# ZhonghuaYi/EI-Nexus_official

Measured on AMD Instinct MI355X. Metric: event-image pairs/s (extract+match, 346x260, 1024 kpts), higher is better.
Workload: dtype f32; 1 GPU; B32 346x260 5-bin event voxel + gray image, VGG(event)+SuperPoint(image) extractors, MNN matcher, k=1024; global_batch=32, event_bins=5, parallelism=dp1 (pairs sharded, metric all-reduce only), log_assignment=False, dense_outputs=False, same_scene_pairs=False, weights=seeded synthetic, descriptor-head bias calibrated (per-channel mean removed)

## Files before the change

### ei-nexus_official_amd/_lib.py

```python
import ctypes
import os

_HERE = os.path.dirname(os.path.abspath(__file__))
LIB_PATH = os.environ.get("EINX_LIB") or os.path.join(_HERE, "libeinx_hip.so")

c_void_p, c_int, c_float, c_size_t, c_char_p = ctypes.c_void_p, ctypes.c_int, ctypes.c_float, ctypes.c_size_t, ctypes.c_char_p


class ConvDesc(ctypes.Structure):
    _fields_ = [("w_native", c_void_p), ("bias", c_void_p), ("scale", c_void_p), ("shift", c_void_p),
                ("cin", ctypes.c_int32), ("cout", ctypes.c_int32), ("ks", ctypes.c_int32), ("relu", ctypes.c_int32),
                ("pool", ctypes.c_int32)]


class DetectParams(ctypes.Structure):
    _fields_ = [("B", ctypes.c_int32), ("Hp", ctypes.c_int32), ("Wp", ctypes.c_int32), ("H", ctypes.c_int32),
                ("W", ctypes.c_int32), ("h0", ctypes.c_int32), ("w0", ctypes.c_int32), ("radius", ctypes.c_int32),
                ("top_k", ctypes.c_int32), ("det_thr", c_float), ("ordering_xy", ctypes.c_int32), ("cap", ctypes.c_int32),
                ("nms_iters", ctypes.c_int32)]


class ExtractorDesc(ctypes.Structure):
    _fields_ = [("struct_size", c_size_t), ("cell", ctypes.c_int32), ("n_backbone", ctypes.c_int32), ("n_det", ctypes.c_int32), ("n_desc", ctypes.c_int32),
                ("backbone", ctypes.POINTER(ConvDesc)), ("det_head", ctypes.POINTER(ConvDesc)), ("desc_head", ctypes.POINTER(ConvDesc)),
# ... 52 lines not shown
                ("match_w", c_void_p), ("match_b", c_void_p), ("n_layers", ctypes.c_int32), ("heads", ctypes.c_int32),
                ("d", ctypes.c_int32), ("input_dim", ctypes.c_int32), ("filter_threshold", c_float),
                ("layers", ctypes.POINTER(LgLayer))]


class LgHead(ctypes.Structure):
    _fields_ = [(n, c_void_p) for n in ("proj_w", "proj_b", "match_w", "match_b", "token_w", "token_b")]


SIGNATURES = {
    "einx_version": (c_char_p, []),
    "einx_abi_version": (c_int, []),
    "einx_build_flags": (c_char_p, []),
    "einx_params_hash": (c_int, [c_void_p, c_int, c_void_p, c_void_p, c_void_p, c_void_p]),
    "einx_last_error": (c_char_p, []),
    "einx_math_eval": (c_int, [c_int, c_void_p, ctypes.c_longlong, c_void_p, c_void_p]),
    "einx_fork_stream_of": (c_void_p, [c_void_p]),
    "einx_fork_stream_prepare_beside": (c_int, [c_void_p, ctypes.POINTER(c_void_p), c_int]),
    "einx_stream_overlap_us": (c_int, [c_void_p, c_void_p, c_int, ctypes.POINTER(ctypes.c_float)]),
    "einx_device_count": (c_int, []),
    "einx_profile_enable": (c_int, [c_int]),
    "einx_profile_report": (c_int, [c_char_p, c_size_t]),
    "einx_extractor_create": (c_void_p, [ctypes.POINTER(ExtractorDesc)]),
    "einx_extractor_destroy": (None, [c_void_p]),
    "einx_fork_stream_prepare": (c_int, [c_void_p]),
    "einx_fork_stream_release": (c_int, [c_void_p]),
    "einx_fork_stream_count": (c_int, []),
    "einx_side_stream": (c_void_p, [c_void_p, c_int, ctypes.POINTER(c_void_p), c_int]),
    "einx_extract_shapes": (c_int, [c_void_p, c_int, c_int, ctypes.POINTER(ExtractShapes)]),
    "einx_extract_ws_bytes": (c_size_t, [c_void_p, c_int, c_int, c_int, c_int, c_int]),
    "einx_extract": (c_int, [c_void_p, c_void_p, c_void_p, c_int, c_int, c_int, c_int, c_void_p, c_size_t, ctypes.POINTER(ExtractOut), c_void_p]),
    "einx_extract_watch": (c_int, [c_void_p, c_void_p, c_void_p, c_int, c_int, c_int, c_int, c_void_p, c_size_t, ctypes.POINTER(ExtractOut),
                           ctypes.POINTER(WeightWatch), c_void_p]),
    "einx_conv_last_kernel": (c_char_p, []),
    "einx_conv_weight_elems": (c_size_t, [c_int, c_int, c_int]),
    "einx_conv_repack": (c_int, [c_void_p, c_int, c_int, c_int, c_void_p, c_void_p]),
    "einx_bn_fold": (c_int, [c_void_p, c_void_p, c_void_p, c_void_p, c_float, c_int, c_void_p, c_void_p, c_void_p]),
    "einx_conv_block": (c_int, [c_void_p, c_int, c_int, c_int, c_int, c_int, c_int, c_int, ctypes.POINTER(ConvDesc), c_void_p, c_void_p]),
    "einx_conv_first_two_fused_ok": (c_int, [ctypes.POINTER(ConvDesc), ctypes.POINTER(ConvDesc), c_int, c_int, c_int]),
    "einx_conv_first_two_fused": (c_int, [c_void_p, c_int, c_int, c_int, c_int, c_int, c_int, c_int, ctypes.POINTER(ConvDesc), ctypes.POINTER(ConvDesc),
                                  c_void_p, c_void_p]),
    "einx_div_inplace": (c_int, [c_void_p, c_size_t, c_float, c_void_p]),
    "einx_image_prepare": (c_int, [c_void_p, c_int, c_int, c_int, c_int, ctypes.c_longlong, ctypes.c_longlong, ctypes.c_longlong, ctypes.c_longlong,
                           c_float, c_void_p, c_void_p]),
    "einx_score_map": (c_int, [c_void_p, c_int, c_int, c_int, c_int, c_void_p, c_int, c_int, c_int, c_int, c_int, c_int, c_void_p,
                               c_void_p, c_void_p]),
    "einx_remove_border": (c_int, [c_void_p, c_int, c_int, c_int, c_int, c_void_p]),
    "einx_detect_ws_bytes": (c_size_t, [ctypes.POINTER(DetectParams)]),
    "einx_detect": (c_int, [c_void_p, ctypes.POINTER(DetectParams), c_void_p, c_void_p, c_void_p, c_void_p, c_void_p, c_void_p,
                            c_void_p, c_void_p]),
    "einx_desc_sample": (c_int, [c_void_p, c_int, c_int, c_int, c_int, c_int, c_int, c_int, c_int, c_void_p, c_void_p, c_int, c_float,
                                 c_void_p, c_void_p]),
    "einx_normalize_map": (c_int, [c_void_p, c_int, c_int, c_int, c_float, c_void_p, c_void_p, c_void_p]),
    "einx_upsample_ws_bytes": (c_size_t, [c_int, c_int, c_int]),
    "einx_upsample_normalize": (c_int, [c_void_p, c_int, c_int, c_int, c_int, c_int, c_int, c_int, c_int, c_int, c_int, c_float,
                                        c_void_p, c_void_p, c_size_t, c_void_p]),
    "einx_mnn_ws_bytes": (c_size_t, [c_int, c_int, c_int]),
    "einx_mnn": (c_int, [c_void_p, c_void_p, c_int, c_void_p, c_void_p, c_int, c_int, c_int, c_void_p, c_void_p, c_void_p, c_void_p,
                         c_void_p, c_void_p, c_void_p]),
    "einx_mnn_gather": (c_int, [c_void_p, c_void_p, c_int, c_void_p, c_void_p, c_int, c_int, c_int, c_void_p, c_void_p, c_void_p, c_void_p,
                                c_void_p, c_void_p, c_void_p, c_void_p, c_int, c_void_p, c_void_p, c_void_p, c_void_p]),
    "einx_mnn_thresh": (c_int, [c_void_p, c_void_p, c_int, c_void_p, c_void_p, c_int, c_int, c_int, c_int, c_float, c_int, c_float, c_void_p,
                                c_void_p, c_void_p, c_void_p, c_void_p, c_void_p, c_void_p]),
    "einx_gather_matches": (c_int, [c_void_p, c_void_p, c_void_p, c_void_p, c_int, c_int, c_int, c_int, c_void_p, c_void_p, c_void_p,
                                    c_void_p]),
    "einx_events_ws_bytes": (c_size_t, [c_int, c_int, c_int]),
    "einx_voxel_ws_bytes": (c_size_t, [c_int, c_int, c_int, c_int, ctypes.c_int64]),
    "einx_voxel_grid": (c_int, [c_void_p, c_void_p, c_void_p, c_void_p, c_void_p, c_int, c_int, c_int, c_int, c_int, c_void_p, c_void_p,
                                c_size_t, c_void_p]),
    "einx_events_mask": (c_int, [c_void_p, c_void_p, c_void_p, c_int, c_int, c_int, c_void_p, c_void_p, c_void_p]),
    "einx_time_surface_ws_bytes": (c_size_t, [c_int, c_int, c_int, c_int, ctypes.c_int64]),
    "einx_event_stack_ws_bytes": (c_size_t, [c_int, c_int, c_int, c_int, ctypes.c_int64]),
    "einx_distance_map_ws_bytes": (c_size_t, [c_int, c_int, c_int, c_int, ctypes.c_int64]),
    "einx_time_surface": (c_int, [c_void_p, c_void_p, c_void_p, c_void_p, c_void_p, c_int, c_int, c_int, c_int, c_void_p, c_void_p, c_size_t,
                                  c_void_p]),
    "einx_event_stack": (c_int, [c_void_p, c_void_p, c_void_p, c_void_p, c_void_p, c_int, c_int, c_int, c_int, c_void_p, c_void_p, c_size_t,
                                 c_void_p]),
    "einx_distance_map": (c_int, [c_void_p, c_void_p, c_void_p, c_void_p, c_void_p, c_int, c_int, c_int, c_int, c_void_p, c_void_p, c_size_t,
                                  c_void_p]),
    "einx_events_pack": (c_int, [ctypes.POINTER(EventArrays), c_int, c_void_p, c_void_p, c_void_p, c_void_p, c_void_p, c_int]),
    "einx_metrics_ws_bytes": (c_size_t, [ctypes.POINTER(MetricParams)]),
    "einx_pair_metrics": (c_int, [ctypes.POINTER(MetricParams)] + [c_void_p] * 13),
    "einx_relative_pose_ws_bytes": (c_size_t, [ctypes.POINTER(PoseParams)]),
    "einx_relative_pose": (c_int, [ctypes.POINTER(PoseParams)] + [c_void_p] * 13),
    "einx_essential_5pt": (c_int, [c_void_p, c_void_p, c_int, c_void_p, c_void_p, c_void_p]),
    "einx_homography_ws_bytes": (c_size_t, [ctypes.POINTER(HomographyParams)]),
    "einx_homography": (c_int, [ctypes.POINTER(HomographyParams)] + [c_void_p] * 11),
    "einx_homography_dlt": (c_int, [c_void_p, c_void_p, c_int, c_int, c_void_p, c_void_p, c_void_p]),
    "einx_gt_matches_ws_bytes": (c_size_t, [ctypes.POINTER(GtMatchesParams)]),
    "einx_gt_project": (c_int, [ctypes.POINTER(GtMatchesParams)] + [c_void_p] * 23),
    "einx_gt_warp": (c_int, [ctypes.POINTER(GtMatchesParams)] + [c_void_p] * 8),
    "einx_gt_label": (c_int, [ctypes.POINTER(GtMatchesParams)] + [c_void_p] * 17),
    "einx_gt_matches": (c_int, [ctypes.POINTER(GtMatchesParams)] + [c_void_p] * 30),
    "einx_match_pr": (c_int, [c_void_p, c_void_p, c_void_p, c_void_p, c_int, c_int, c_void_p, c_void_p]),
    "einx_desc_loss_ws_bytes": (c_size_t, [c_int] * 11),
    "einx_desc_loss": (c_int, [c_void_p, c_float, c_void_p, c_float] + [c_int] * 11 + [c_void_p, c_int, c_int, c_void_p, c_void_p, c_size_t, c_void_p]),
    "einx_map_loss_ws_bytes": (c_size_t, [c_int, c_int]),
    "einx_map_loss": (c_int, [c_void_p, c_void_p, c_int, c_int, c_int, c_void_p, c_int, c_int, c_int, c_void_p, c_void_p, c_size_t, c_void_p]),
    "einx_logits_loss": (c_int, [c_void_p, c_void_p] + [c_int] * 9 + [c_void_p, c_int, c_void_p, c_void_p, c_size_t, c_void_p]),
    "einx_linear": (c_int, [c_void_p, c_int, c_int, c_void_p, c_void_p, c_int, c_void_p, c_int, c_void_p]),
    "einx_lg_ws_bytes": (c_size_t, [c_int, c_int, c_int, c_int, c_int]),
    "einx_lg_ws_bytes_heads": (c_size_t, [c_int, c_int, c_int, c_int, c_int, c_int]),
    "einx_lightglue": (c_int, [ctypes.POINTER(LgWeights), c_void_p, c_void_p, c_void_p, c_int, c_void_p, c_void_p, c_void_p, c_int,
                               c_int, c_float, c_float, c_float, c_float, c_void_p, c_void_p, c_void_p, c_void_p, c_void_p, c_void_p,
                               c_void_p, c_void_p, c_int, c_void_p]),
    "einx_lightglue_early_stop_ws_bytes": (c_size_t, [c_int] * 7),
# ... 48 lines not shown
```

### ei-nexus_official_amd/_native.py

```python
import ctypes
import threading
import os
import math

import numpy as np
import torch

from . import _lib
from ._lib import ConvDesc, DetectParams, check

F32 = torch.float32


def lib():
    return _lib.load()


I32, I64, U8 = torch.int32, torch.int64, torch.uint8


def _dev_check(*tensors, dt=F32):
    for t in tensors:
        if t is None:
            continue
# ... 192 lines not shown

class Detection:
    __slots__ = ("positions", "indices", "counts", "thr", "not_converged", "nms", "cap", "padded", "pads", "stale")


def detect(score, *, top_k, radius, det_thr, pads=(0, 0, 0, 0), ordering="yx", cap=None, nms_iters=8, want_nms=True):
    _dev_check(score)
    B = score.shape[0]
    Hp, Wp = score.shape[-2:]
    w0, w1, h0, h1 = pads
    H, W = Hp - h0 - h1, Wp - w0 - w1
    N = Hp * Wp
    if cap is None:
        cap = topk_capacity(N, top_k, det_thr)
    cap = max(int(cap), 1)
    p = DetectParams(B, Hp, Wp, H, W, h0, w0, int(radius), int(top_k or 0), float(det_thr), int(ordering == "xy"), cap, int(nms_iters))
    L = lib()
    dev = score.device
    ws = _workspace(L.einx_detect_ws_bytes(ctypes.byref(p)), dev)
    d = Detection()
    d.positions = torch.empty((B, cap, 3), dtype=F32, device=dev)
    d.indices = torch.empty((B, cap), dtype=torch.int32, device=dev)
    d.counts = torch.empty((B,), dtype=torch.int32, device=dev)
    d.thr = torch.empty((B,), dtype=F32, device=dev)
    d.not_converged = torch.empty((B,), dtype=torch.int32, device=dev)
    d.nms = torch.empty((B, H, W), dtype=F32, device=dev) if want_nms else None
    d.cap, d.padded, d.pads = cap, (Hp, Wp), pads
    check(L.einx_detect(_ptr(score), ctypes.byref(p), _ptr(ws), _ptr(d.nms), _ptr(d.positions), _ptr(d.indices), _ptr(d.counts),
                        _ptr(d.thr), _ptr(d.not_converged), _stream(score)), "einx_detect")
    return d


def desc_sample(raw, indices, counts, padded_size, bilinear, scale, raw_cl=None):
    _dev_check(raw, raw_cl)
    _dev_check(indices, counts, dt=I32)
    B, D, hc, wc = raw.shape
    cap = indices.shape[1]
    out = torch.empty((B, cap, D), dtype=F32, device=raw.device)
    use_cl = raw_cl is not None and bilinear
    src = raw_cl if use_cl else raw
    check(lib().einx_desc_sample(_ptr(src), B, D, hc, wc, int(padded_size[0]), int(padded_size[1]), int(bilinear), int(use_cl),
                                 _ptr(indices), _ptr(counts), cap, float(scale), _ptr(out), _stream(raw)), "einx_desc_sample")
    return out


def normalize_map(raw, scale, want_cl=False):
    _dev_check(raw)
    B, D = raw.shape[:2]
    P = int(raw.numel() // (B * D))
    out = torch.empty_like(raw)
    cl = torch.empty((B, P, D), dtype=F32, device=raw.device) if (want_cl and D <= 512) else None
    check(lib().einx_normalize_map(_ptr(raw), B, D, P, float(scale), _ptr(out), _ptr(cl), _stream(raw)), "einx_normalize_map")
    return (out, cl) if want_cl else out


def upsample_normalize(raw, padded_size, pads, scale):
    _dev_check(raw)
    B, D, hc, wc = raw.shape
    Hp, Wp = int(padded_size[0]), int(padded_size[1])
    w0, w1, h0, h1 = pads
    H, W = Hp - h0 - h1, Wp - w0 - w1
    out = torch.empty((B, D, H, W), dtype=F32, device=raw.device)
    nws = int(lib().einx_upsample_ws_bytes(B, H, W))
    ws = torch.empty((nws + 3) // 4, dtype=F32, device=raw.device)
    check(lib().einx_upsample_normalize(_ptr(raw), B, D, hc, wc, Hp, Wp, h0, w0, H, W, float(scale), _ptr(out), _ptr(ws), nws, _stream(raw)),
          "einx_upsample_normalize")
    return out


class MatchResult:
    __slots__ = ("matches0", "matches1", "scores0", "scores1", "la", "mk0", "mk1", "nmatch", "ref0", "ref1", "mk0_flat", "mk1_flat", "stale", "stop")

    def __init__(self):
        self.mk0_flat = self.mk1_flat = None
        self.stale = None
        self.stop = None


def mnn(desc0, n, desc1, m, want_la=True, ratio_thresh=None, distance_thresh=None, gather=None):
    _dev_check(desc0, desc1)
    _dev_check(n, m, dt=I32)
    B, cap0, D = desc0.shape
    cap1 = desc1.shape[1]
    L = lib()
    dev = desc0.device
    ws = _workspace(L.einx_mnn_ws_bytes(B, cap0, cap1), dev)
    r = MatchResult()
    r.matches0 = torch.empty((B, cap0), dtype=torch.int64, device=dev)
    r.matches1 = torch.empty((B, cap1), dtype=torch.int64, device=dev)
    r.scores0 = torch.empty((B, cap0), dtype=F32, device=dev)
    r.scores1 = torch.empty((B, cap1), dtype=F32, device=dev)
    r.la = torch.empty((B, cap0 + 1, cap1 + 1), dtype=F32, device=dev) if want_la else None
    r.ref0 = r.ref1 = None
    if ratio_thresh or distance_thresh:
        r2 = float(np.float32(float(ratio_thresh) ** 2)) if ratio_thresh else 0.0
        t2 = float(np.float32(float(distance_thresh) ** 2)) if distance_thresh else 0.0
        check(L.einx_mnn_thresh(_ptr(desc0), _ptr(n), cap0, _ptr(desc1), _ptr(m), cap1, B, D, int(bool(ratio_thresh)), r2,
                                int(bool(distance_thresh)), t2, _ptr(ws), _ptr(r.matches0), _ptr(r.matches1), _ptr(r.scores0), _ptr(r.scores1),
                                _ptr(r.la), _stream(desc0)), "einx_mnn_thresh")
        return r if gather is None else gather_matches(r, gather[0], gather[1], n, gather[2])
    if gather is not None:
        k0, k1, cols = gather
        _dev_check(k0, k1)
        r.mk0 = torch.empty((B, cap0, cols), dtype=F32, device=dev)
        r.mk1 = torch.empty((B, cap0, cols), dtype=F32, device=dev)
        r.nmatch = torch.empty((B,), dtype=torch.int32, device=dev)
# ... 293 lines not shown
```

### ei-nexus_official_amd/csrc/extract.hip

```cpp
#include <stdlib.h>
#include <string.h>

#include <algorithm>
#include <mutex>
#include <new>
#include <vector>

#include "einx_common.h"

struct einx_extractor {
  einx_extractor_desc d;
  std::vector<einx_conv_desc> backbone, det, desc;
  bool has_merged = false;
  einx_conv_desc merged;
};

namespace {

struct Plan {
  int Hp, Wp, h0, w0;
  int hc, wc;
  size_t buf_elems[2];
  size_t head_elems;
};
// ... 182 lines not shown
                                   size_t ws_bytes, const einx_extract_out* o, const einx_weight_watch* ww, void* stream) {
  EINX_CHECK_ARG(e && in && ws && o, "null pointer");
  EINX_CHECK_ARG(!ww || ww->struct_size == sizeof(einx_weight_watch), "einx_weight_watch::struct_size does not match this library (ABI mismatch)");
  EINX_CHECK_ARG(!ww || ww->n == 0 || (ww->n > 0 && ww->table && ww->ref && ww->scratch && ww->stale), "weight watch with null pointers");
  EINX_CHECK_ARG(o->feats && o->logits && o->raw && o->prob && o->score && o->positions && o->indices && o->counts && o->thr &&
                     o->not_converged && o->sparse_desc,
                 "null output pointer");
  EINX_CHECK_ARG(B > 0 && H > 0 && W > 0 && o->cap > 0, "bad shape");
  Plan pl;
  EINX_CHECK_ARG(make_plan(e, H, W, &pl), "image size does not fit the network's pooling / cell size");
  EINX_CHECK_ARG(e->d.cell == 1 || (o->coarse && o->raw_cl), "cell-8 networks need the coarse / raw_cl outputs");
  EINX_CHECK_ARG(ws_bytes >= einx_extract_ws_bytes(e, B, H, W, o->cap, nms_iters), "workspace smaller than einx_extract_ws_bytes for these arguments");
  einx_detect_params dp;
  detect_params(e, pl, B, H, W, o->cap, nms_budget(nms_iters), &dp);
  WsCarver c{(char*)ws};
  const ExtractWs wk = carve(c, e, pl, &dp, B);
  bool fork = fork_heads(e, pl, B) && !einx_profile_active();
  {
    hipStreamCaptureStatus cs = hipStreamCaptureStatusNone;
    if (fork && hipStreamIsCapturing((hipStream_t)stream, &cs) == hipSuccess && cs != hipStreamCaptureStatusNone) fork = false;
  }
  float* const head2 = fork ? wk.head2 : wk.head;
  int rc;
  if (e->d.input_div != 0.0f && e->d.input_div != 1.0f) {
    rc = einx_div_inplace(in, (size_t)B * e->backbone.front().cin * H * W, e->d.input_div, stream);
    if (rc) return rc;
  }
  const float* cur = in;
  int h = pl.Hp, w = pl.Wp;
  const int nb = (int)e->backbone.size();
  int first = 0;
  if (nb >= 2 && 1 == einx_conv_first_two_fused_ok(&e->backbone[0], &e->backbone[1], B, pl.Hp, pl.Wp)) {
    float* out = (2 < nb) ? wk.buf[1] : o->feats;
    if ((rc = einx_conv_first_two_fused(in, B, H, W, pl.h0, pl.w0, pl.Hp, pl.Wp, &e->backbone[0], &e->backbone[1], out, stream))) return rc;
    if (e->backbone[1].pool) {
      h /= 2;
      w /= 2;
    }
    cur = out;
    first = 2;
  }
  for (int i = first; i < nb; ++i) {
    const einx_conv_desc& c = e->backbone[i];
    float* out = (i + 1 < nb) ? wk.buf[i & 1] : o->feats;
    if (i == 0) rc = einx_conv_block(cur, B, H, W, pl.h0, pl.w0, pl.Hp, pl.Wp, &c, out, stream);
    else rc = einx_conv_block(cur, B, h, w, 0, 0, h, w, &c, out, stream);
    if (rc) return rc;
    if (c.pool) {
      h /= 2;
      w /= 2;
    }
    cur = out;
  }
  auto run_head = [&](const std::vector<einx_conv_desc>& L, float* scratch, float* final_out, void* st) -> int {
    const float* x = o->feats;
    for (size_t i = 0; i < L.size(); ++i) {
      float* out = (i + 1 < L.size()) ? scratch : final_out;
      const int r = einx_conv_block(x, B, h, w, 0, 0, h, w, &L[i], out, st);
      if (r) return r;
      x = out;
    }
    return 0;
  };
  const int D = e->desc.back().cout;
  const bool merged = e->has_merged && B == 1;
  if (merged && (rc = einx_conv_block(o->feats, B, h, w, 0, 0, h, w, &e->merged, wk.head, stream))) return rc;
  const float* desc_in = wk.head + (size_t)e->det.front().cout * h * w;
  auto det_branch = [&](void* st) -> int {
    if (merged) return einx_conv_block(wk.head, B, h, w, 0, 0, h, w, &e->det[1], o->logits, st);
    return run_head(e->det, wk.head, o->logits, st);
  };
  auto desc_branch = [&](void* st) -> int {
    int r = merged ? einx_conv_block(desc_in, B, h, w, 0, 0, h, w, &e->desc[1], o->raw, st) : run_head(e->desc, head2, o->raw, st);
    if (r) return r;
    if (e->d.cell == 8) r = einx_normalize_map(o->raw, B, D, h * w, e->d.desc_scale, o->coarse, o->raw_cl, st);
    return r;
  };
  std::unique_lock<std::mutex> side_lock;
  const EinxSide* sd = fork ? einx_side_acquire((hipStream_t)stream, &side_lock) : nullptr;
  if (sd) {
    if (hipEventRecord(sd->fork, (hipStream_t)stream) != hipSuccess || hipStreamWaitEvent(sd->stream, sd->fork, 0) != hipSuccess) {
      einx_set_error("einx_extract: fork failed");
      return EINX_ERR_LAUNCH;
    }
    rc = desc_branch(sd->stream);
    const bool ok = hipEventRecord(sd->join, sd->stream) == hipSuccess;
    if (rc) {
      (void)hipStreamWaitEvent((hipStream_t)stream, sd->join, 0);
      return rc;
    }
    if (!ok) {
      einx_set_error("einx_extract: join failed");
      return EINX_ERR_LAUNCH;
    }
    if ((rc = det_branch(stream))) {
      (void)hipStreamWaitEvent((hipStream_t)stream, sd->join, 0);
      return rc;
    }
  } else {
    if ((rc = det_branch(stream))) return rc;
    if ((rc = desc_branch(stream))) return rc;
  }
  const int C_det = e->det.back().cout;
  const long score_threads = (long)(C_det == 65 ? einx_cdiv(B * h * w, 32) : einx_cdiv(B * h * w, 256)) * 256;
  const bool zero_in_score = wk.det.nflags > 0 && wk.det.nflags <= score_threads;
  rc = einx_score_map_zero(o->logits, B, C_det, h, w, mask, H, W, pl.h0, pl.w0, e->d.dilate_mask, e->d.border, o->prob, o->score,
                           zero_in_score ? wk.det.flags : nullptr, zero_in_score ? wk.det.nflags : 0, o->score_crop, stream);
  if (rc) {
    if (sd) (void)hipStreamWaitEvent((hipStream_t)stream, sd->join, 0);
    return rc;
  }
  const float* nms_map = nullptr;
  rc = einx_detect_prezeroed(o->score, &dp, wk.det_ws, o->nms, o->positions, o->indices, o->counts, o->thr, o->not_converged, zero_in_score ? 1 : 0,
                             o->nms ? &nms_map : nullptr, stream);
  if (sd && hipStreamWaitEvent((hipStream_t)stream, sd->join, 0) != hipSuccess && !rc) {
    einx_set_error("einx_extract: join failed");
    return EINX_ERR_LAUNCH;
  }
  if (rc) return rc;
  const bool bilinear = e->d.cell == 8;
  const bool use_cl = bilinear && D <= 512;
  EinxWatch watch;
  const bool on = ww && ww->n > 0;
  watch.table = on ? ww->table : nullptr;
  watch.ref = on ? (const unsigned long long*)ww->ref : nullptr;
  watch.hash = on ? (unsigned long long*)ww->scratch : nullptr;
  watch.flag = on ? ww->stale : nullptr;
  watch.n = on ? ww->n : 0;
  watch.bit = 1;
  EinxCrop crop{};
  crop.map = o->nms ? nms_map : nullptr;
  crop.thr = o->thr;
  crop.out = o->nms;
  crop.Hp = pl.Hp;
  crop.Wp = pl.Wp;
  crop.h0 = pl.h0;
  crop.w0 = pl.w0;
  crop.H = H;
  crop.W = W;
  return einx_desc_sample_watch(use_cl ? o->raw_cl : o->raw, B, D, h, w, pl.Hp, pl.Wp, bilinear ? 1 : 0, use_cl ? 1 : 0, o->indices, o->counts,
                                o->cap, e->d.desc_scale, o->sparse_desc, watch, crop, stream);
}
```

### include/einx.h

```cpp
#ifndef EINX_H
#define EINX_H

#include <stddef.h>
#include <stdint.h>

#ifdef __cplusplus
extern "C" {
#endif

#define EINX_OK 0
#define EINX_ERR_ARG (-1)
#define EINX_ERR_LAUNCH (-2)
#define EINX_ERR_NO_DEVICE (-3)

#define EINX_ABI_VERSION 6
int einx_abi_version(void);
const char* einx_version(void);
const char* einx_last_error(void);
const char* einx_build_flags(void);
int einx_device_count(void);

#define EINX_WATCH_CHUNK_WORDS 4096
int einx_params_hash(const int64_t* table, int n, uint64_t* hash, const uint64_t* ref, int32_t* stale, void* stream);

// ... 14 lines not shown
typedef struct einx_conv_desc {
  const float* w_native;
  const float* bias;
  const float* scale;
  const float* shift;
  int32_t cin, cout, ks;
  int32_t relu;
  int32_t pool;
} einx_conv_desc;

int einx_conv_block(const float* in, int B, int Hs, int Ws, int h0, int w0, int H, int W, const einx_conv_desc* d, float* out,
                    void* stream);

int einx_conv_first_two_fused_ok(const einx_conv_desc* d0, const einx_conv_desc* d1, int B, int H, int W);
int einx_conv_first_two_fused(const float* in, int B, int Hs, int Ws, int h0, int w0, int H, int W, const einx_conv_desc* d0,
                              const einx_conv_desc* d1, float* out, void* stream);

const char* einx_conv_last_kernel(void);

int einx_div_inplace(float* x, size_t n, float divisor, void* stream);

int einx_image_prepare(float* image, int B, int C, int H, int W, long long stride_b, long long stride_c, long long stride_h,
                       long long stride_w, float divisor, float* gray, void* stream);


int einx_score_map(const float* logits, int B, int C, int hc, int wc, const uint8_t* mask, int H, int W, int h0, int w0,
                   int dilate, int border, float* prob, float* score, void* stream);

int einx_remove_border(float* score, int B, int Hp, int Wp, int border, void* stream);

int einx_dense_positions(const float* score, int B, int H, int W, int ordering_xy, float* out, void* stream);

typedef struct einx_detect_params {
  int32_t B, Hp, Wp;
  int32_t H, W, h0, w0;
  int32_t radius;
  int32_t top_k;
  float det_thr;
  int32_t ordering_xy;
  int32_t cap;
  int32_t nms_iters;
} einx_detect_params;

size_t einx_detect_ws_bytes(const einx_detect_params* p);

int einx_detect(const float* score, const einx_detect_params* p, void* ws, float* nms_out, float* positions, int32_t* indices,
                int32_t* counts, float* thr, int32_t* not_converged, void* stream);


int einx_desc_sample(const float* raw, int B, int D, int hc, int wc, int Hp, int Wp, int bilinear, int channels_last,
                     const int32_t* indices, const int32_t* counts, int cap, float scale, float* out, void* stream);

int einx_normalize_map(const float* raw, int B, int D, int P, float scale, float* out, float* raw_cl, void* stream);

int einx_normalize_rows(const float* x, int R, int C, float scale, float* out, void* stream);

int einx_random_positions(const float* u, int R, float size0, float size1, float* out, void* stream);

size_t einx_upsample_ws_bytes(int B, int H, int W);
int einx_upsample_normalize(const float* raw, int B, int D, int hc, int wc, int Hp, int Wp, int h0, int w0, int H, int W,
                            float scale, float* out, void* ws, size_t ws_bytes, void* stream);

size_t einx_mnn_ws_bytes(int B, int cap0, int cap1);
int einx_mnn(const float* desc0, const int32_t* n, int cap0, const float* desc1, const int32_t* m, int cap1, int B, int D,
             void* ws, int64_t* matches0, int64_t* matches1, float* scores0, float* scores1, float* la, void* stream);
int einx_mnn_gather(const float* desc0, const int32_t* n, int cap0, const float* desc1, const int32_t* m, int cap1, int B, int D,
                    void* ws, int64_t* matches0, int64_t* matches1, float* scores0, float* scores1, float* la, const float* kpts0,
                    const float* kpts1, int cols, float* mk0, float* mk1, int32_t* nmatch, void* stream);
int einx_mnn_thresh(const float* desc0, const int32_t* n, int cap0, const float* desc1, const int32_t* m, int cap1, int B, int D,
                    int use_ratio, float ratio_sq, int use_dist, float dist_sq, void* ws, int64_t* matches0, int64_t* matches1,
                    float* scores0, float* scores1, float* la, void* stream);

int einx_similarity(const float* desc0, const int32_t* n, int cap0, const float* desc1, const int32_t* m, int cap1, int B, int D,
                    float* sim, void* stream);

int einx_gather_matches(const float* kpts0, const float* kpts1, const int64_t* matches0, const int32_t* n, int cap0, int cap1,
                        int B, int cols, float* out0, float* out1, int32_t* nmatch, void* stream);

int einx_compact_rows(const float* src0, const float* src1, const int32_t* counts, int B, int cap, int width, float* dst0, float* dst1,
                      void* stream);

int einx_linear(const float* x, int M, int K, const float* w, const float* bias, int N, float* y, int accumulate, void* stream);

typedef struct einx_lg_layer {
  const float *Wqkv, *bqkv, *Wo, *bo, *sf0_w, *sf0_b, *sln_g, *sln_b, *sf3_w, *sf3_b;
  const float *Wqk, *bqk, *Wv, *bv, *Wco, *bco, *cf0_w, *cf0_b, *cln_g, *cln_b, *cf3_w, *cf3_b;
  const float *Wqk_v, *bqk_v;
} einx_lg_layer;

typedef struct einx_lg_weights {
  size_t struct_size;
  size_t layer_size;
  const float* in_w;
  const float* in_b;
  const float* Wr;
  const float* proj_w;
  const float* proj_b;
  const float* match_w;
  const float* match_b;
  int32_t n_layers, heads, d, input_dim;
  float filter_threshold;
  const einx_lg_layer* layers;
} einx_lg_weights;

int einx_normalize_keypoints(const float* kpts, int rows, int cols, float h, float w, float* out, int out_cols, void* stream);

// ... 214 lines not shown
```

Before: 3753 pairs/s.

## Fuse final 1x1 head convs with softmax score map and descriptor normalization

Adds new HIP kernels that compute the last 1x1 conv of the detector head (65 channels) with MFMA and, in the same kernel, do the per-cell softmax, masking, border removal and depth-to-space score map. A second kernel fuses the last descriptor-head 1x1 conv (256 channels) with L2 normalization and writes the channels-last copy. By default (env var set to 1) only the detector fusion is on; the descriptor fusion needs the env var set to 2. The goal is to drop the separate score-map pass and the extra round trip of logits through global memory. In exchange the fused kernel uses fixed tiles and an LDS-heavy epilogue that may reach lower occupancy than the generic conv.

```diff
diff --git a/ei-nexus_official_amd/_lib.py b/ei-nexus_official_amd/_lib.py
--- a/ei-nexus_official_amd/_lib.py
+++ b/ei-nexus_official_amd/_lib.py
@@ -128,6 +128,11 @@
     "einx_desc_sample": (c_int, [c_void_p, c_int, c_int, c_int, c_int, c_int, c_int, c_int, c_int, c_void_p, c_void_p, c_int, c_float,
                                  c_void_p, c_void_p]),
     "einx_normalize_map": (c_int, [c_void_p, c_int, c_int, c_int, c_float, c_void_p, c_void_p, c_void_p]),
+    "einx_head_det_score_ok": (c_int, [ctypes.POINTER(ConvDesc)]),
+    "einx_head_det_score": (c_int, [c_void_p, c_int, c_int, c_int, ctypes.POINTER(ConvDesc), c_void_p, c_int, c_int, c_int, c_int, c_int, c_int,
+                                    c_void_p, c_void_p, c_void_p, c_void_p, c_int, c_void_p, c_void_p]),
+    "einx_head_desc_normalize_ok": (c_int, [ctypes.POINTER(ConvDesc)]),
+    "einx_head_desc_normalize": (c_int, [c_void_p, c_int, c_int, ctypes.POINTER(ConvDesc), c_float, c_void_p, c_void_p, c_void_p, c_void_p]),
     "einx_upsample_ws_bytes": (c_size_t, [c_int, c_int, c_int]),
     "einx_upsample_normalize": (c_int, [c_void_p, c_int, c_int, c_int, c_int, c_int, c_int, c_int, c_int, c_int, c_int, c_float,
                                         c_void_p, c_void_p, c_size_t, c_void_p]),
diff --git a/ei-nexus_official_amd/_native.py b/ei-nexus_official_amd/_native.py
--- a/ei-nexus_official_amd/_native.py
+++ b/ei-nexus_official_amd/_native.py
@@ -268,6 +268,44 @@
     cl = torch.empty((B, P, D), dtype=F32, device=raw.device) if (want_cl and D <= 512) else None
     check(lib().einx_normalize_map(_ptr(raw), B, D, P, float(scale), _ptr(out), _ptr(cl), _stream(raw)), "einx_normalize_map")
     return (out, cl) if want_cl else out
+
+
+def head_det_score(x, layer, mask=None, pads=(0, 0, 0, 0), dilate=False, border=0, want_crop=True):
+    _dev_check(x)
+    if mask is not None and mask.device.type != "cuda":
+        raise RuntimeError(f"einx: the mask must live on a HIP device, got {mask.device}")
+    B, C, hc, wc = x.shape
+    if C != layer.cin:
+        raise ValueError(f"conv expects {layer.cin} input channels, got {C}")
+    Hp, Wp = hc * 8, wc * 8
+    w0, w1, h0, h1 = pads
+    H, W = Hp - h0 - h1, Wp - w0 - w1
+    logits = torch.empty((B, 65, hc, wc), dtype=F32, device=x.device)
+    prob = torch.empty_like(logits)
+    score = torch.empty((B, 1, Hp, Wp), dtype=F32, device=x.device)
+    crop = torch.empty((B, 1, H, W), dtype=F32, device=x.device) if want_crop else None
+    m8 = None
+    if mask is not None:
+        if tuple(mask.shape[-2:]) != (H, W):
+            raise ValueError(f"mask spatial size {tuple(mask.shape[-2:])} does not match the image ({H},{W})")
+        m8 = (mask if mask.dtype == torch.bool else mask.ne(0)).contiguous().view(torch.uint8)
+    check(lib().einx_head_det_score(_ptr(x), B, hc, wc, ctypes.byref(layer.desc), _ptr(m8), H, W, h0, w0, int(dilate), int(border), _ptr(logits),
+                                    _ptr(prob), _ptr(score), None, 0, _ptr(crop), _stream(x)), "einx_head_det_score")
+    return logits, prob, score, crop
+
+
+def head_desc_normalize(x, layer, scale):
+    _dev_check(x)
+    B, C, hc, wc = x.shape
+    if C != layer.cin:
+        raise ValueError(f"conv expects {layer.cin} input channels, got {C}")
+    P = hc * wc
+    raw = torch.empty((B, layer.cout, hc, wc), dtype=F32, device=x.device)
+    coarse = torch.empty_like(raw)
+    cl = torch.empty((B, P, layer.cout), dtype=F32, device=x.device)
+    check(lib().einx_head_desc_normalize(_ptr(x), B, P, ctypes.byref(layer.desc), float(scale), _ptr(raw), _ptr(coarse), _ptr(cl), _stream(x)),
+          "einx_head_desc_normalize")
+    return raw, coarse, cl
 
 
 def upsample_normalize(raw, padded_size, pads, scale):
diff --git a/ei-nexus_official_amd/csrc/extract.hip b/ei-nexus_official_amd/csrc/extract.hip
--- a/ei-nexus_official_amd/csrc/extract.hip
+++ b/ei-nexus_official_amd/csrc/extract.hip
@@ -258,26 +258,51 @@
     }
     cur = out;
   }
-  auto run_head = [&](const std::vector<einx_conv_desc>& L, float* scratch, float* final_out, void* st) -> int {
+  auto run_head = [&](const std::vector<einx_conv_desc>& L, size_t n, float* scratch, float* final_out, void* st, const float** last) -> int {
     const float* x = o->feats;
-    for (size_t i = 0; i < L.size(); ++i) {
+    for (size_t i = 0; i < n; ++i) {
       float* out = (i + 1 < L.size()) ? scratch : final_out;
       const int r = einx_conv_block(x, B, h, w, 0, 0, h, w, &L[i], out, st);
       if (r) return r;
       x = out;
     }
+    if (last) *last = x;
     return 0;
   };
   const int D = e->desc.back().cout;
+  const char* hf_env = getenv("EINX_HEADS_FUSED");
+  const int hf = e->d.cell != 8 ? 0 : (hf_env && hf_env[0] >= '0' && hf_env[0] <= '2' ? hf_env[0] - '0' : 1);
+  const bool det_fused = hf >= 1 && einx_head_det_score_ok(&e->det.back());
+  const bool desc_fused = hf >= 2 && einx_head_desc_normalize_ok(&e->desc.back());
+  const int C_det = e->det.back().cout;
+  const long score_threads = det_fused ? (long)B * einx_cdiv(h * w, 64) * 256 : (long)(C_det == 65 ? einx_cdiv(B * h * w, 32) : einx_cdiv(B * h * w, 256)) * 256;
+  const bool zero_in_score = wk.det.nflags > 0 && wk.det.nflags <= score_threads;
   const bool merged = e->has_merged && B == 1;
   if (merged && (rc = einx_conv_block(o->feats, B, h, w, 0, 0, h, w, &e->merged, wk.head, stream))) return rc;
   const float* desc_in = wk.head + (size_t)e->det.front().cout * h * w;
   auto det_branch = [&](void* st) -> int {
+    if (det_fused) {
+      const float* x = wk.head;
+      if (!merged) {
+        const int r = run_head(e->det, e->det.size() - 1, wk.head, o->logits, st, &x);
+        if (r) return r;
+      }
+      return einx_head_det_score(x, B, h, w, &e->det.back(), mask, H, W, pl.h0, pl.w0, e->d.dilate_mask, e->d.border, o->logits, o->prob, o->score,
+                                 zero_in_score ? wk.det.flags : nullptr, zero_in_score ? wk.det.nflags : 0, o->score_crop, st);
+    }
     if (merged) return einx_conv_block(wk.head, B, h, w, 0, 0, h, w, &e->det[1], o->logits, st);
-    return run_head(e->det, wk.head, o->logits, st);
+    return run_head(e->det, e->det.size(), wk.head, o->logits, st, nullptr);
   };
   auto desc_branch = [&](void* st) -> int {
-    int r = merged ? einx_conv_block(desc_in, B, h, w, 0, 0, h, w, &e->desc[1], o->raw, st) : run_head(e->desc, head2, o->raw, st);
+    if (desc_fused) {
+      const float* x = desc_in;
+      if (!merged) {
+        const int r = run_head(e->desc, e->desc.size() - 1, head2, o->raw, st, &x);
+        if (r) return r;
+      }
+      return einx_head_desc_normalize(x, B, h * w, &e->desc.back(), e->d.desc_scale, o->raw, o->coarse, o->raw_cl, st);
+    }
+    int r = merged ? einx_conv_block(desc_in, B, h, w, 0, 0, h, w, &e->desc[1], o->raw, st) : run_head(e->desc, e->desc.size(), head2, o->raw, st, nullptr);
     if (r) return r;
     if (e->d.cell == 8) r = einx_normalize_map(o->raw, B, D, h * w, e->d.desc_scale, o->coarse, o->raw_cl, st);
     return r;
@@ -307,11 +332,9 @@
     if ((rc = det_branch(stream))) return rc;
     if ((rc = desc_branch(stream))) return rc;
   }
-  const int C_det = e->det.back().cout;
-  const long score_threads = (long)(C_det == 65 ? einx_cdiv(B * h * w, 32) : einx_cdiv(B * h * w, 256)) * 256;
-  const bool zero_in_score = wk.det.nflags > 0 && wk.det.nflags <= score_threads;
-  rc = einx_score_map_zero(o->logits, B, C_det, h, w, mask, H, W, pl.h0, pl.w0, e->d.dilate_mask, e->d.border, o->prob, o->score,
-                           zero_in_score ? wk.det.flags : nullptr, zero_in_score ? wk.det.nflags : 0, o->score_crop, stream);
+  rc = det_fused ? EINX_OK
+                 : einx_score_map_zero(o->logits, B, C_det, h, w, mask, H, W, pl.h0, pl.w0, e->d.dilate_mask, e->d.border, o->prob, o->score,
+                                       zero_in_score ? wk.det.flags : nullptr, zero_in_score ? wk.det.nflags : 0, o->score_crop, stream);
   if (rc) {
     if (sd) (void)hipStreamWaitEvent((hipStream_t)stream, sd->join, 0);
     return rc;
diff --git a/ei-nexus_official_amd/csrc/heads.hip b/ei-nexus_official_amd/csrc/heads.hip
--- /dev/null
+++ b/ei-nexus_official_amd/csrc/heads.hip
@@ -0,0 +1,412 @@
+#include "einx_common.h"
+
+namespace {
+
+constexpr int HD_CK = 32;
+constexpr int HD_PX = 64;
+
+struct HeadConv {
+  const float* in;
+  const float* w;
+  const float* bias;
+  const float* scale;
+  const float* shift;
+  int Cin, P, CoutPad, relu, runs;
+};
+
+struct HeadDetArgs {
+  HeadConv c;
+  float* logits;
+  const uint8_t* mask;
+  int hc, wc, H, W, h0, w0, dilate, border;
+  float* prob;
+  float* score;
+  int32_t* zero_ptr;
+  int zero_n;
+  float* crop;
+};
+
+constexpr int DET_PITCH = HD_PX + 1;
+
+__global__ __launch_bounds__(256, 3) void head_det_score_kernel(const HeadDetArgs a) {
+  constexpr int IN_LDS = HD_CK * HD_PX, W_LDS = HD_CK * 64;
+  constexpr int STAGE = IN_LDS + W_LDS + HD_CK, TILE = 65 * DET_PITCH;
+  __shared__ __attribute__((aligned(16))) float lds[STAGE > TILE ? STAGE : TILE];
+  __shared__ float s_bias[65], s_scale[65], s_shift[65];
+  float* in_tile = lds;
+  float* w_tile = lds + IN_LDS;
+  float* wx_tile = lds + IN_LDS + W_LDS;
+
+  const int tid = threadIdx.x;
+  if ((int)(blockIdx.x * 256 + tid) < a.zero_n) a.zero_ptr[blockIdx.x * 256 + tid] = 0;
+  const int wave = __builtin_amdgcn_readfirstlane(tid >> 6);
+  const int wm = wave >> 1, wn = wave & 1;
+  const int lane = tid & 63, half = lane >> 5, j = lane & 31;
+  const int b = (int)blockIdx.x / a.c.runs, p0 = ((int)blockIdx.x % a.c.runs) * HD_PX;
+  const int P = a.c.P, CP = a.c.CoutPad;
+  if (tid < 65) {
+    s_bias[tid] = a.c.bias ? a.c.bias[tid] : 0.0f;
+    s_scale[tid] = a.c.scale ? a.c.scale[tid] : 1.0f;
+    s_shift[tid] = a.c.scale ? a.c.shift[tid] : 0.0f;
+  }
+  const int pos = tid & 63, grp = tid >> 6;
+  const float* src = a.c.in + (size_t)b * a.c.Cin * P + min(p0 + pos, P - 1) + (size_t)grp * 8 * P;
+  const float* wsrc = a.c.w + (size_t)(tid >> 4) * CP + (tid & 15) * 4;
+  float r_in[8];
+  f32x4 r_w[2];
+  float r_wx = 0.0f;
+  auto issue_loads = [&](int c) {
+    const float* s = src + (size_t)c * HD_CK * P;
+#pragma unroll
+    for (int i = 0; i < 8; ++i) r_in[i] = s[(size_t)i * P];
+    const float* wc_ = wsrc + (size_t)c * HD_CK * CP;
+    r_w[0] = *reinterpret_cast<const f32x4*>(wc_);
+    r_w[1] = *reinterpret_cast<const f32x4*>(wc_ + (size_t)16 * CP);
+    if (tid < HD_CK) r_wx = a.c.w[(size_t)(c * HD_CK + tid) * CP + 64];
+  };
+  auto commit_loads = [&]() {
+#pragma unroll
+    for (int i = 0; i < 8; ++i) in_tile[(grp * 8 + i) * HD_PX + pos] = r_in[i];
+    *reinterpret_cast<f32x4*>(w_tile + tid * 4) = r_w[0];
+    *reinterpret_cast<f32x4*>(w_tile + (tid + 256) * 4) = r_w[1];
+    if (tid < HD_CK) wx_tile[tid] = r_wx;
+  };
+  f32x16 acc;
+#pragma unroll
+  for (int r = 0; r < 16; ++r) acc[r] = 0.0f;
+  float xacc = 0.0f;
+  const int aBase = half * 64 + wm * 32 + j, bBase = half * HD_PX + wn * 32 + j;
+  const int nchunks = a.c.Cin / HD_CK;
+  issue_loads(0);
+  for (int c = 0; c < nchunks; ++c) {
+    __syncthreads();
+    commit_loads();
+    __syncthreads();
+    if (c + 1 < nchunks) issue_loads(c + 1);
+    constexpr int STEPS = HD_CK / 2, PF = 2;
+    float av[PF + 1], bv[PF + 1];
+#pragma unroll
+    for (int st = 0; st < PF; ++st) {
+      av[st] = w_tile[aBase + st * 2 * 64];
+      bv[st] = in_tile[bBase + st * 2 * HD_PX];
+    }
+#pragma unroll
+    for (int st = 0; st < STEPS; ++st) {
+      if (st + PF < STEPS) {
+        av[(st + PF) % (PF + 1)] = w_tile[aBase + (st + PF) * 2 * 64];
+        bv[(st + PF) % (PF + 1)] = in_tile[bBase + (st + PF) * 2 * HD_PX];
+      }
+      __builtin_amdgcn_sched_barrier(0);
+      acc = __builtin_amdgcn_mfma_f32_32x32x2f32(av[st % (PF + 1)], bv[st % (PF + 1)], acc, 0, 0, 0);
+      __builtin_amdgcn_sched_barrier(0);
+    }
+    if (tid < HD_PX) {
+#pragma unroll
+      for (int r = 0; r < HD_CK; ++r) xacc = fmaf(wx_tile[r], in_tile[r * HD_PX + tid], xacc);
+    }
+  }
+  __syncthreads();
+
+  float* lg = a.logits + (size_t)b * 65 * P;
+  {
+    const int q = wn * 32 + j;
+    const bool st_ok = p0 + q < P;
+#pragma unroll
+    for (int r = 0; r < 16; ++r) {
+      const int ch = wm * 32 + 8 * (r >> 2) + 4 * half + (r & 3);
+      float v = acc[r] + s_bias[ch];
+      if (a.c.relu) v = fmaxf(v, 0.0f);
+      if (a.c.scale) v = fmaf(v, s_scale[ch], s_shift[ch]);
+      if (st_ok) lg[(size_t)ch * P + p0 + q] = v;
+      lds[ch * DET_PITCH + q] = v;
+    }
+  }
+  if (tid < HD_PX) {
+    float v = xacc + s_bias[64];
+    if (a.c.relu) v = v > 0.0f ? v : 0.0f;
+    if (a.c.scale) v = fmaf(v, s_scale[64], s_shift[64]);
+    if (p0 + tid < P) lg[(size_t)64 * P + p0 + tid] = v;
+    lds[64 * DET_PITCH + tid] = v;
+  }
+  __syncthreads();
+
+  const int cells = P, hc = a.hc, wc = a.wc, H = a.H, W = a.W, h0 = a.h0, w0 = a.w0, dilate = a.dilate, border = a.border;
+  const uint8_t* mask = a.mask;
+  const int jj = lane & 7, i = lane >> 3;
+#pragma unroll 1
+  for (int pass = 0; pass < 2; ++pass) {
+    const int lc = pass * 32 + wave * 8 + jj;
+    const int cell = p0 + lc;
+    const bool valid = cell < cells;
+    float v[8];
+#pragma unroll
+    for (int k = 0; k < 8; ++k) v[k] = lds[(8 * i + k) * DET_PITCH + lc];
+    const float v64 = lds[64 * DET_PITCH + lc];
+    float mx = v64;
+#pragma unroll
+    for (int k = 0; k < 8; ++k) mx = fmaxf(mx, v[k]);
+    mx = fmaxf(mx, __shfl_xor(mx, 8, 64));
+    mx = fmaxf(mx, __shfl_xor(mx, 16, 64));
+    mx = fmaxf(mx, __shfl_xor(mx, 32, 64));
+    float e[8];
+#pragma unroll
+    for (int k = 0; k < 8; ++k) e[k] = einx_expf(v[k] - mx);
+    const float e64 = einx_expf(v64 - mx);
+    float s = 0.0f;
+#pragma unroll
+    for (int c = 0; c < 64; ++c) s = s + __shfl(e[c & 7], jj + 8 * (c >> 3), 64);
+    s = s + e64;
+    if (!valid) continue;
+    const int h = cell / wc, w = cell % wc;
+    const int Hp = hc * 8, Wp = wc * 8;
+    float* pr = a.prob + (size_t)b * 65 * cells + cell;
+    const int y = h * 8 + i;
+    unsigned cols = 0x3ffu;
+    if (mask) {
+      cols = 0;
+      const int r = dilate ? 1 : 0;
+#pragma unroll
+      for (int dy = -1; dy <= 1; ++dy) {
+        const int yy = y + dy, sy = yy - h0;
+        const bool rok = dy >= -r && dy <= r && yy >= 0 && yy < Hp && sy >= 0 && sy < H;
+        const uint8_t* mrow = mask + ((size_t)b * H + min(max(sy, 0), H - 1)) * W;
+        uint8_t m[10];
+#pragma unroll
+        for (int k = 0; k < 10; ++k) m[k] = mrow[min(max(w * 8 - 1 + k - w0, 0), W - 1)];
+#pragma unroll
+        for (int k = 0; k < 10; ++k) {
+          const int xx = w * 8 - 1 + k, sx = xx - w0;
+          if (rok && xx >= 0 && xx < Wp && sx >= 0 && sx < W && m[k]) cols |= 1u << k;
+        }
+      }
+    }
+    const unsigned window = (mask && !dilate) ? 2u : 7u;
+    float out[8];
+#pragma unroll
+    for (int k = 0; k < 8; ++k) {
+      const float p = e[k] / s;
+      pr[(size_t)(8 * i + k) * cells] = p;
+      const int x = w * 8 + k;
+      float t = p;
+      if (!((cols >> k) & window)) t = 0.0f;
+      if (border > 0 && (y < border || y >= Hp - border || x < border || x >= Wp - border)) t = 0.0f;
+      out[k] = t;
+    }
+    if (i == 0) pr[(size_t)64 * cells] = e64 / s;
+    f32x4* dst = reinterpret_cast<f32x4*>(a.score + ((size_t)b * Hp + y) * Wp + w * 8);
+    dst[0] = f32x4{out[0], out[1], out[2], out[3]};
+    dst[1] = f32x4{out[4], out[5], out[6], out[7]};
+    if (a.crop) {
+      const int uy = y - h0;
+      if (uy >= 0 && uy < H) {
+        float* cr = a.crop + ((size_t)b * H + uy) * W - w0 + w * 8;
+#pragma unroll
+        for (int k = 0; k < 8; ++k) {
+          const int ux = w * 8 + k - w0;
+          if (ux >= 0 && ux < W) cr[k] = out[k];
+        }
+      }
+    }
+  }
+}
+
+struct HeadDescArgs {
+  HeadConv c;
+  float scale;
+  float* raw;
+  float* coarse;
+  float* raw_cl;
+};
+
+template <int D>
+__global__ __launch_bounds__(256, 2) void head_desc_norm_kernel(const HeadDescArgs a) {
+  constexpr int PT = HD_PX;
+  constexpr int MT = D / 128;
+  static_assert(D % 128 == 0 && D * PT * 4 <= 65536, "tile must fit the static LDS limit");
+  constexpr int IN_LDS = HD_CK * PT, W_F4 = HD_CK * D / 4, W_PER_THR = W_F4 / 256;
+  static_assert(IN_LDS + HD_CK * D <= D * PT, "staging aliases the tile");
+  __shared__ __attribute__((aligned(16))) float lds[D * PT];
+  float* in_tile = lds;
+  float* w_tile = lds + IN_LDS;
+
+  const int tid = threadIdx.x;
+  const int wave = __builtin_amdgcn_readfirstlane(tid >> 6);
+  const int lane = tid & 63, half = lane >> 5, j = lane & 31;
+  const int b = (int)blockIdx.x / a.c.runs, p0 = ((int)blockIdx.x % a.c.runs) * PT;
+  const int P = a.c.P;
+  const int px = tid % PT, cgrp = tid / PT;
+  const bool pv = p0 + px < P;
+  const float* src = a.c.in + (size_t)b * a.c.Cin * P + (pv ? p0 + px : P - 1) + (size_t)cgrp * 8 * P;
+  const float* wsrc = a.c.w + tid * 4;
+  float r_in[8];
+  f32x4 r_w[W_PER_THR];
+  auto issue_loads = [&](int c) {
+    const float* s = src + (size_t)c * HD_CK * P;
+#pragma unroll
+    for (int i = 0; i < 8; ++i) r_in[i] = s[(size_t)i * P];
+    const float* wc_ = wsrc + (size_t)c * HD_CK * D;
+#pragma unroll
+    for (int i = 0; i < W_PER_THR; ++i) r_w[i] = *reinterpret_cast<const f32x4*>(wc_ + (size_t)i * 1024);
+  };
+  auto commit_loads = [&]() {
+#pragma unroll
+    for (int i = 0; i < 8; ++i) in_tile[(cgrp * 8 + i) * PT + px] = r_in[i];
+#pragma unroll
+    for (int i = 0; i < W_PER_THR; ++i) *reinterpret_cast<f32x4*>(w_tile + (tid + i * 256) * 4) = r_w[i];
+  };
+  f32x16 acc[MT][2];
+#pragma unroll
+  for (int mt = 0; mt < MT; ++mt)
+#pragma unroll
+    for (int nt = 0; nt < 2; ++nt)
+#pragma unroll
+      for (int r = 0; r < 16; ++r) acc[mt][nt][r] = 0.0f;
+  const int aBase = half * D + wave * (MT * 32) + j, bBase = half * PT + j;
+  const int nchunks = a.c.Cin / HD_CK;
+  issue_loads(0);
+  for (int c = 0; c < nchunks; ++c) {
+    __syncthreads();
+    commit_loads();
+    __syncthreads();
+    if (c + 1 < nchunks) issue_loads(c + 1);
+    constexpr int STEPS = HD_CK / 2, PF = 2;
+    float av[PF + 1][MT], bv[PF + 1][2];
+    auto load_frag = [&](int st, int buf) {
+#pragma unroll
+      for (int mt = 0; mt < MT; ++mt) av[buf][mt] = w_tile[aBase + st * 2 * D + mt * 32];
+#pragma unroll
+      for (int nt = 0; nt < 2; ++nt) bv[buf][nt] = in_tile[bBase + st * 2 * PT + nt * 32];
+    };
+#pragma unroll
+    for (int st = 0; st < PF; ++st) load_frag(st, st);
+#pragma unroll
+    for (int st = 0; st < STEPS; ++st) {
+      if (st + PF < STEPS) load_frag(st + PF, (st + PF) % (PF + 1));
+      __builtin_amdgcn_sched_barrier(0);
+#pragma unroll
+      for (int mt = 0; mt < MT; ++mt)
+#pragma unroll
+        for (int nt = 0; nt < 2; ++nt)
+          acc[mt][nt] = __builtin_amdgcn_mfma_f32_32x32x2f32(av[st % (PF + 1)][mt], bv[st % (PF + 1)][nt], acc[mt][nt], 0, 0, 0);
+      __builtin_amdgcn_sched_barrier(0);
+    }
+  }
+  __syncthreads();
+
+  float* rb = a.raw + (size_t)b * D * P;
+#pragma unroll
+  for (int mt = 0; mt < MT; ++mt)
+#pragma unroll
+    for (int r = 0; r < 16; ++r) {
+      const int ch = wave * (MT * 32) + mt * 32 + 8 * (r >> 2) + 4 * half + (r & 3);
+      const float bi = a.c.bias ? a.c.bias[ch] : 0.0f;
+      const float sc = a.c.scale ? a.c.scale[ch] : 1.0f;
+      const float sh = a.c.scale ? a.c.shift[ch] : 0.0f;
+#pragma unroll
+      for (int nt = 0; nt < 2; ++nt) {
+        const int q = nt * 32 + j;
+        float v = acc[mt][nt][r] + bi;
+        if (a.c.relu) v = fmaxf(v, 0.0f);
+        if (a.c.scale) v = fmaf(v, sc, sh);
+        if (p0 + q < P) rb[(size_t)ch * P + p0 + q] = v;
+        lds[ch * PT + ((q + ch) & (PT - 1))] = v;
+      }
+    }
+  __syncthreads();
+
+  float s = 0.0f;
+  for (int c = 0; c + 16 <= D; c += 16) {
+    float v[16];
+#pragma unroll
+    for (int u = 0; u < 16; ++u) v[u] = lds[(c + u) * PT + ((px + c + u) & (PT - 1))];
+#pragma unroll
+    for (int u = 0; u < 16; ++u) s = fmaf(v[u], v[u], s);
+  }
+  const float den = fmaxf(sqrtf(s), 1e-12f);
+  if (pv) {
+    constexpr int CG = 256 / PT;
+    float* ob = a.coarse + (size_t)b * D * P + p0 + px;
+    for (int c = cgrp; c + 3 * CG < D; c += 4 * CG) {
+      float v[4];
+#pragma unroll
+      for (int u = 0; u < 4; ++u) v[u] = a.scale * (lds[(c + u * CG) * PT + ((px + c + u * CG) & (PT - 1))] / den);
+#pragma unroll
+      for (int u = 0; u < 4; ++u) ob[(size_t)(c + u * CG) * P] = v[u];
+    }
+  }
+  if (a.raw_cl) {
+    float* cb = a.raw_cl + ((size_t)b * P + p0) * D;
+    const int npx = min(PT, P - p0);
+    for (int pixel = wave; pixel < npx; pixel += 4) {
+      float* cp = cb + (size_t)pixel * D;
+#pragma unroll
+      for (int c = lane; c < D; c += 64) cp[c] = lds[c * PT + ((pixel + c) & (PT - 1))];
+    }
+  }
+}
+
+bool head_layer_fits(const einx_conv_desc* d) { return d && d->w_native && d->ks == 1 && !d->pool && d->cin > 0 && d->cin % HD_CK == 0; }
+
+}
+
+EINX_EXPORT int einx_head_det_score_ok(const einx_conv_desc* d) { return head_layer_fits(d) && d->cout == 65; }
+
+EINX_EXPORT int einx_head_desc_normalize_ok(const einx_conv_desc* d) { return head_layer_fits(d) && d->cout == 256; }
+
+EINX_EXPORT int einx_head_det_score(const float* in, int B, int hc, int wc, const einx_conv_desc* d, const uint8_t* mask, int H, int W, int h0, int w0,
+                                    int dilate, int border, float* logits, float* prob, float* score, int32_t* zero_ptr, int zero_n, float* crop,
+                                    void* stream) {
+  EINX_CHECK_ARG(in && d && logits && prob && score, "null pointer");
+  EINX_CHECK_ARG(einx_head_det_score_ok(d), "layer outside what the fused detector head covers (1x1, cout 65, cin a multiple of 32, no pool)");
+  EINX_CHECK_ARG((d->scale == nullptr) == (d->shift == nullptr), "scale and shift go together");
+  EINX_CHECK_ARG(B > 0 && hc > 0 && wc > 0, "bad shape");
+  EINX_CHECK_ARG(!(crop || mask) || (H > 0 && W > 0), "the mask and the cropped map need the un-padded size");
+  EINX_CHECK_ARG((size_t)d->cin * hc * wc < (1u << 30), "image too large (2^30 elements per image and tensor)");
+  const int P = hc * wc, runs = einx_cdiv(P, HD_PX);
+  EINX_CHECK_ARG((long)B * runs < (1L << 22), "batch too large");
+  EINX_CHECK_ARG(zero_n == 0 || (zero_ptr && (long)zero_n <= (long)B * runs * 256), "more words to zero than threads in the launch");
+  HeadDetArgs a;
+  a.c = HeadConv{in, d->w_native, d->bias, d->scale, d->shift, d->cin, P, 128, d->relu, runs};
+  a.logits = logits;
+  a.mask = mask;
+  a.hc = hc;
+  a.wc = wc;
+  a.H = H;
+  a.W = W;
+  a.h0 = h0;
+  a.w0 = w0;
+  a.dilate = dilate;
+  a.border = border;
+  a.prob = prob;
+  a.score = score;
+  a.zero_ptr = zero_ptr;
+  a.zero_n = zero_n;
+  a.crop = crop;
+  hipStream_t s = (hipStream_t)stream;
+  EINX_PROF("conv_block_kernel 1x1 + score map (det head)", s);
+  hipLaunchKernelGGL(head_det_score_kernel, dim3((unsigned)(B * runs)), dim3(256), 0, s, a);
+  EINX_CHECK_LAUNCH();
+  return EINX_OK;
+}
+
+EINX_EXPORT int einx_head_desc_normalize(const float* in, int B, int P, const einx_conv_desc* d, float scale, float* raw, float* coarse, float* raw_cl,
+                                         void* stream) {
+  EINX_CHECK_ARG(in && d && raw && coarse, "null pointer");
+  EINX_CHECK_ARG(einx_head_desc_normalize_ok(d), "layer outside what the fused descriptor head covers (1x1, cout 256, cin a multiple of 32, no pool)");
+  EINX_CHECK_ARG((d->scale == nullptr) == (d->shift == nullptr), "scale and shift go together");
+  EINX_CHECK_ARG(B > 0 && P > 0, "bad shape");
+  EINX_CHECK_ARG((size_t)d->cin * P < (1u << 30) && (size_t)d->cout * P < (1u << 30), "image too large (2^30 elements per image and tensor)");
+  const int runs = einx_cdiv(P, HD_PX);
+  EINX_CHECK_ARG((long)B * runs < (1L << 22), "batch too large");
+  HeadDescArgs a;
+  a.c = HeadConv{in, d->w_native, d->bias, d->scale, d->shift, d->cin, P, 256, d->relu, runs};
+  a.scale = scale;
+  a.raw = raw;
+  a.coarse = coarse;
+  a.raw_cl = raw_cl;
+  hipStream_t s = (hipStream_t)stream;
+  EINX_PROF("conv_block_kernel 1x1 + normalize (desc head)", s);
+  hipLaunchKernelGGL(head_desc_norm_kernel<256>, dim3((unsigned)(B * runs)), dim3(256), 0, s, a);
+  EINX_CHECK_LAUNCH();
+  return EINX_OK;
+}
diff --git a/include/einx.h b/include/einx.h
--- a/include/einx.h
+++ b/include/einx.h
@@ -90,6 +90,14 @@
                      const int32_t* indices, const int32_t* counts, int cap, float scale, float* out, void* stream);
 
 int einx_normalize_map(const float* raw, int B, int D, int P, float scale, float* out, float* raw_cl, void* stream);
+
+int einx_head_det_score_ok(const einx_conv_desc* d);
+int einx_head_det_score(const float* in, int B, int hc, int wc, const einx_conv_desc* d, const uint8_t* mask, int H, int W, int h0, int w0,
+                        int dilate, int border, float* logits, float* prob, float* score, int32_t* zero_ptr, int zero_n, float* crop,
+                        void* stream);
+int einx_head_desc_normalize_ok(const einx_conv_desc* d);
+int einx_head_desc_normalize(const float* in, int B, int P, const einx_conv_desc* d, float scale, float* raw, float* coarse, float* raw_cl,
+                             void* stream);
 
 int einx_normalize_rows(const float* x, int R, int C, float scale, float* out, void* stream);
 
```

Measured after the change: 3774 pairs/s (median of 4 runs). No clear change (+0.5%).
